# crowdbotp/socialways

Measured on AMD Instinct MI355X. Metric: GAN train steps/sec (256 scenes x 8 agents x 8+12 T per GPU step; fp32; social block on), higher is better.
Workload: dtype f32; 1 GPU; m1: 256 scenes x 8 agents x (8 obs + 12 pred) per GPU step = reference --batch-size 2048; use_social=True, n_unrolling_steps=1, info loss on; full=False, global_batch_scenes=256, parallelism=dp1, steps_per_graph_launch=32, settle_steps=992, rehearsal_regions=2, step_alg_bytes=5527040, inputs=z drawn on the host every step

## Files before the change

### socialways_amd/csrc/sw_disc.hip

```cpp
#include "../../include/socialways_hip.h"
#include "sw_lstm_dev.h"
#include "sw_wgrad.h"
#include "sw_wgrad_dev.h"
#include <cstdlib>
#ifdef SW_PHASE_STAMPS
__device__ long long sw_disc_stamps[16];
#define SW_STAMP(k) do { __builtin_amdgcn_sched_barrier(0); long long _t = clock64(); if (blockIdx.x == 0 && threadIdx.x == 0) sw_disc_stamps[k] += _t - _tprev; _tprev = _t; __builtin_amdgcn_sched_barrier(0); } while (0)
#define SW_STAMP_INIT long long _tprev = clock64()
extern "C" int sw_debug_disc_stamps(long long* out, int reset) {
  if (reset) { long long z[16] = {0}; return (int)hipMemcpyToSymbol(HIP_SYMBOL(sw_disc_stamps), z, sizeof(z)); }
  return (int)hipMemcpyFromSymbol(out, HIP_SYMBOL(sw_disc_stamps), 16 * sizeof(long long));
}
#else
#define SW_STAMP(k)
#define SW_STAMP_INIT
#endif

#define SW_DSTAMP(k) SW_STAMP(k)
#define SW_DSTAMP_INIT SW_STAMP_INIT
#include "sw_disc_dev.h"

__global__ __launch_bounds__(SW_THREADS, 2) void disc_fwd_kernel(
    const float* __restrict__ obsv, int To, int x_mode, const float* __restrict__ pred_a,
    const float* __restrict__ pred_b, int nb, const float* __restrict__ d_w, int B, int Tp, float* __restrict__ label_a, float* __restrict__ label_b,
    float* __restrict__ code_a, float* __restrict__ code_b, float* __restrict__ dsave, int save_lstm, int split,
    float* __restrict__ w_snap, int fuse, DiscLoss gl, float* __restrict__ dpred_out, const float* __restrict__ dimg) {
  extern __shared__ __attribute__((aligned(16))) float smem[];
  disc_fwd_tile(smem, blockIdx.x, gridDim.x, obsv, To, x_mode, pred_a, pred_b, nb, d_w, B, Tp, label_a, label_b, code_a, code_b, dsave,
                save_lstm, split, w_snap, fuse, gl, dpred_out, dimg);
}

#define SW_SPLIT_MAX_WGS 256

__global__ __launch_bounds__(SW_THREADS, 2) void disc_bwd_kernel(
    const float* __restrict__ d_w, const float* __restrict__ dsave, const float* __restrict__ dlabel_a,
    const float* __restrict__ dlabel_b, const float* __restrict__ dcode_a, const float* __restrict__ dcode_b, int nb,
    int B, int To, int Tp, int want_w, float* __restrict__ ddelta, float* __restrict__ dpred_a,
    float* __restrict__ dpred_b, DiscLoss gl, const float* __restrict__ dimg) {
  extern __shared__ __attribute__((aligned(16))) float smem[];
  const HeadLdsB L = head_lds_b(Tp, 0);
  float* dgbuf = smem + L.pe0T;
  const swp::Disc O = swp::disc(Tp);
  const DSave ds = dsave_layout(B, To, Tp, nb);
  const DDelta dd = ddelta_layout(B, To, Tp, nb);
  const int lane = sw_lane(), wave = sw_wave(), ln = lane & 15, lg = lane >> 4;
  const int u0 = wave * 16;
  const int a0 = blockIdx.x * SW_TILE;
  const int b = min(a0 + ln, B - 1);
  const bool live = (a0 + ln) < B;
  const int K4 = 4 * Tp;

  SW_STAMP_INIT;
  const int m0h = 16 * (wave & 1);
  f32x4 pc1[2], pq1[2], po1;
#pragma unroll
  for (int k = 0; k < 2; ++k) {
    const size_t kb = (size_t)min(k, nb - 1) * B + b;
    pc1[k] = ld4(dsave + (wave < 2 ? ds.c1 : ds.l1) + kb * 32 + m0h + 4 * lg);
    pq1[k] = ld4(dsave + ds.q1 + kb * 32 + m0h + 4 * lg);
  }
  po1 = ld4(dsave + ds.o1 + (size_t)b * 32 + m0h + 4 * lg);
  float hl[2][2], hc[2][2], hz[2], htg[2], rl[2], rc[2], rz[2];
  {
    const float* zsrc = gl.on ? gl.z : dsave;
    const float* tsrc = gl.on ? gl.targets : dsave;
    htg[0] = tsrc[gl.on ? gl.t0 : 0];
    htg[1] = tsrc[gl.on ? gl.t1 : 0];
    const float* dl1 = nb > 1 ? dlabel_b : dlabel_a;
    const float* dc1p = nb > 1 ? dcode_b : dcode_a;
#pragma unroll
    for (int e = 0; e < 2; ++e) {
      const int i = min((int)threadIdx.x + SW_THREADS * e, 16 * LD16 - 1);
      const int a = i / LD16, c1 = min(i - a * LD16, 1);
      const int bb = min(a0 + a, B - 1);
      hl[e][0] = dlabel_a[bb];
      hl[e][1] = dl1[bb];
      hc[e][0] = dcode_a[(size_t)bb * 2 + c1];
      hc[e][1] = dc1p[(size_t)bb * 2 + c1];
      hz[e] = zsrc[(size_t)bb * SW_Z + c1];
    }
    const int bb = min(a0 + ln, B - 1);
    rl[0] = dlabel_a[bb];
    rl[1] = dl1[bb];
    rc[0] = dcode_a[(size_t)bb * 2];
    rc[1] = dcode_a[(size_t)bb * 2 + 1];
    rz[0] = zsrc[(size_t)bb * SW_Z];
    rz[1] = zsrc[(size_t)bb * SW_Z + 1];
  }
  for (int i = threadIdx.x; i < 16 * LD32; i += blockDim.x) smem[L.docode + i] = 0.f;
  disc_stage_headT(smem, L, true, d_w, O, K4, dimg, true, [&] {
    stage_zero(smem + L.of0T, L.dlab - L.of0T);
    sw_barrier();
  });

  for (int k = 0; k < nb; ++k) {
    float* dpred = k == 0 ? dpred_a : dpred_b;
    sw_barrier();
    if (k == 0) SW_STAMP(8);
#pragma unroll
    for (int e = 0; e < 2; ++e) {
      const int i = threadIdx.x + SW_THREADS * e;
      if (i < 16 * LD16) {
        const int a = i / LD16, cc = i - a * LD16;
        const int bb = min(a0 + a, B - 1);
        const float xl = k == 0 ? hl[e][0] : hl[e][1], xc = k == 0 ? hc[e][0] : hc[e][1];
        float vl, vc;
        if (gl.on) {
          const float tgt = k == 0 ? htg[0] : htg[1];
          vl = cc == 0 ? 2.0f * (xl - tgt) * gl.g_label : 0.f;
          vc = (k == 0 && cc < 2) ? 2.0f * (xc - hz[e]) * gl.g_code : 0.f;
        } else {
          vl = cc == 0 ? xl : 0.f;
          vc = cc < 2 ? xc : 0.f;
        }
        smem[L.dlab + i] = vl;
        smem[L.dcod + i] = vc;
        if (want_w && a0 + a < B && cc < 4) {
          ddelta[dd.dlab + ((size_t)k * B + bb) * 4 + cc] = vl;
          ddelta[dd.dcod + ((size_t)k * B + bb) * 4 + cc] = vc;
        }
      }
    }
    if (gl.on && gl.loss_part && wave == 3 && k < 2) {
      const bool lv = lane < 16 && a0 + lane < B;
      const float e = (k == 0 ? rl[0] : rl[1]) - (k == 0 ? htg[0] : htg[1]);
      float sl = lv ? e * e : 0.f, sc = 0.f;
      if (k == 0 && lv) {
        const float c0 = rc[0] - rz[0], c1 = rc[1] - rz[1];
        sc = c0 * c0 + c1 * c1;
      }
#pragma unroll
      for (int o = 8; o > 0; o >>= 1) {
        sl += __shfl_xor(sl, o);
        sc += __shfl_xor(sc, o);
      }
      if (lane == 0) {
        gl.loss_part[(size_t)blockIdx.x * 3 + (k == 0 ? 0 : 2)] = sl;
        if (k == 0) gl.loss_part[(size_t)blockIdx.x * 3 + 1] = sc;
      }
    }
    sw_barrier();
    {
      int m0 = 16 * (wave & 1);
      bool cls = wave < 2;
      f32x4 acc = {0.f, 0.f, 0.f, 0.f};
      acc = tile_mm_rt(smem + (cls ? L.cl1T : L.la1T) + (m0 + ln) * LD16 + 4 * lg,
                       smem + (cls ? L.dlab : L.dcod) + ln * LD16 + 4 * lg, 1, acc);
      const f32x4 a = k == 0 ? pc1[0] : pc1[1];
#pragma unroll
      for (int r = 0; r < 4; ++r) acc[r] = sw_lrelu_grad(a[r], acc[r]);
      st4(smem + (cls ? L.dc1 : L.dl1) + ln * LD32 + m0 + 4 * lg, acc);
      if (want_w && live) st4(ddelta + (cls ? dd.dc1 : dd.dl1) + ((size_t)k * B + b) * 32 + m0 + 4 * lg, acc);
    }
    sw_barrier();
    {
      f32x4 acc = {0.f, 0.f, 0.f, 0.f};
      acc = tile_mm_rt(smem + L.cl0T + (u0 + ln) * LD32 + 4 * lg, smem + L.dc1 + ln * LD32 + 4 * lg, 2, acc);
      acc = tile_mm_rt(smem + L.la0T + (u0 + ln) * LD32 + 4 * lg, smem + L.dl1 + ln * LD32 + 4 * lg, 2, acc);
      st4(smem + L.dboth + ln * LD64 + u0 + 4 * lg, acc);
      if (wave < 2) {
        float* p = smem + L.docode + ln * LD32 + u0 + 4 * lg;
        st4(p, ld4(p) + acc);
      } else if (want_w && live) {
        st4(ddelta + dd.dpcode + ((size_t)k * B + b) * 32 + (u0 - 32) + 4 * lg, acc);
      }
    }
    sw_barrier();
    if (wave < 2) {
      int m0 = 16 * wave;
      f32x4 acc = {0.f, 0.f, 0.f, 0.f};
      acc = tile_mm_rt(smem + L.pe1T + (m0 + ln) * LD32 + 4 * lg, smem + L.dboth + ln * LD64 + 32 + 4 * lg, 2, acc);
      const f32x4 a = k == 0 ? pq1[0] : pq1[1];
#pragma unroll
      for (int r = 0; r < 4; ++r) acc[r] = sw_lrelu_grad(a[r], acc[r]);
      st4(smem + L.dq1 + ln * LD32 + m0 + 4 * lg, acc);
      if (want_w && live) st4(ddelta + dd.dq1 + ((size_t)k * B + b) * 32 + m0 + 4 * lg, acc);
    }
    sw_barrier();
    if (dpred) {
      for (int mt = wave; mt * 16 < K4; mt += 4) {
        int m0 = 16 * mt;
        f32x4 acc = {0.f, 0.f, 0.f, 0.f};
        acc = tile_mm_rt(smem + L.pe0T + (m0 + ln) * LD32 + 4 * lg, smem + L.dq1 + ln * LD32 + 4 * lg, 2, acc);
        if (live && m0 + 4 * lg < K4) st4(dpred + (size_t)b * K4 + m0 + 4 * lg, acc);
      }
    }
  }
  if (!want_w) return;
  sw_barrier();
  SW_STAMP(9);
  if (live && wave < 2) st4(ddelta + dd.docode + (size_t)b * 32 + u0 + 4 * lg, ld4(smem + L.docode + ln * LD32 + u0 + 4 * lg));
  f32x4 dh = disc_obs_bwd_tail(smem + L.of1T, smem + L.of0T, smem + L.docode, smem + L.do1, po1, ddelta + dd.do1 + (size_t)b * 32, live);
  f32x4 dc = {0.f, 0.f, 0.f, 0.f};
  LstmWT WT;
  lstm_load_whhT(WT, dimg, swdimg::OP_WHHT, d_w + O.whh, wave, lane);
  const LstmBptt S{dsave + ds.act + (size_t)b * 384 + u0 + 4 * lg, nullptr, dgbuf, ddelta + dd.dgates + (size_t)a0 * 256,
                   ddelta + dd.trash, a0, B};
  lstm_bptt_rows<false>(WT, S, To, dh, dc, SwNop{}, [&](int k) { SW_STAMP(k); });
}

namespace {
struct UpdLds {
  int hbuf, hw, bias, hwT, x, q1, both, c1, l1, o1, total;
  int dlab, dcod, dc1, dl1, dboth, docode, do1, dend;
  int ldp;
  HeadLds F;
  HeadLdsB T;
};
__host__ __device__ inline UpdLds upd_lds(int Tp) {
  UpdLds U;
  U.F = head_lds(Tp, 0);
  U.T = head_lds_b(Tp, 0);
  U.ldp = U.F.ldp;
  int o = 0;
  U.hbuf = o; o += 2 * 16 * SW_HLD;
  U.hw = o; o += U.F.bias - U.F.of0;
  U.bias = o; o += 8 * 32;
  U.hwT = o; o += U.T.dlab - U.T.of0T;
  U.x = o; o += 2 * 16 * U.ldp;
  U.q1 = o; o += 2 * 16 * LD32;
  U.both = o; o += 2 * 16 * LD64;
  U.c1 = o; o += 2 * 16 * LD32;
  U.l1 = o; o += 2 * 16 * LD32;
  U.o1 = o; o += 16 * LD32;
  U.total = o;
  int d = U.hw;
  U.dlab = d; d += 2 * 16 * LD16;
  U.dcod = d; d += 2 * 16 * LD16;
  U.dc1 = d; d += 2 * 16 * LD32;
  U.dl1 = d; d += 2 * 16 * LD32;
  U.dboth = d; d += 2 * 16 * LD64;
  U.docode = d; d += 16 * LD32;
  U.do1 = d; d += 16 * LD32;
  U.dend = d;
  return U;
}
}

__global__ __launch_bounds__(SW_THREADS) void disc_update_kernel(
    const float* __restrict__ obsv, int To, const float* __restrict__ pred_a, const float* __restrict__ pred_b,
    const float* __restrict__ d_w, int B, int Tp, float* __restrict__ label_a, float* __restrict__ label_b,
    float* __restrict__ code_a, float* __restrict__ code_b, float* __restrict__ dsave, int obs_pre, float* __restrict__ w_snap,
    DiscLoss gl, float* __restrict__ ddelta, const float* __restrict__ dimg) {
  extern __shared__ __attribute__((aligned(16))) float smem[];
  const UpdLds U = upd_lds(Tp);
  const HeadLds& F = U.F;
  const HeadLdsB& T = U.T;
  const swp::Disc O = swp::disc(Tp);
  const DSave ds = dsave_layout(B, To, Tp, 2);
  const DDelta dd = ddelta_layout(B, To, Tp, 2);
  float* hbuf = smem + U.hbuf;
  const int lane = sw_lane(), wave = sw_wave(), ln = lane & 15, lg = lane >> 4;
  const int u0 = wave * 16, br = wave >> 1, wp = wave & 1;
  const int a0 = blockIdx.x * SW_TILE;
  const int b = min(a0 + ln, B - 1);
  const bool live = (a0 + ln) < B;
  const int K4 = 4 * Tp, ldp = U.ldp;
  float* hw = smem + U.hw - F.of0;
  float* hwT = smem + U.hwT - T.of0T;

  float xpre[2][4];
  disc_xpre_load(xpre, pred_a, pred_b, a0, B, K4, ldp);
  const float tg0 = gl.targets[gl.t0], tg1 = gl.targets[gl.t1];
  const float z0 = gl.z[(size_t)b * SW_Z], z1 = gl.z[(size_t)b * SW_Z + 1];
  LstmW W;
  if (!obs_pre) disc_obs_operands(W, d_w, O, dimg);
  if (w_snap)
    for (int i = blockIdx.x * SW_THREADS + threadIdx.x; i < O.n; i += gridDim.x * SW_THREADS) w_snap[i] = d_w[i];
  disc_stage_heads(hw, F, d_w, O, K4, true);
  disc_stage_headT(hwT, T, true, nullptr, O, K4, dimg, false);
#pragma unroll
  for (int kk = 0; kk < 2; ++kk)
    disc_xpre_put(xpre, kk == 1, smem + U.x + kk * 16 * ldp, dsave + ds.px + (size_t)kk * B * K4, a0, B, K4, ldp);
  f32x4 c = {0.f, 0.f, 0.f, 0.f}, h = {0.f, 0.f, 0.f, 0.f};
  disc_seed_h(hbuf, obs_pre, dsave + ds.act, To, B, b);
  sw_barrier();
  const bool reg8 = !obs_pre && To == 8;
  f32x4 sg[8][4], sc[8];
  if (reg8) {
    float xa, xq;
    obs_x4_load(obsv, b, 0, 8, lg, xa, xq);
    asm volatile("" : "+v"(xa), "+v"(xq));
    float* hrow_g = dsave + ds.act + (size_t)b * 384 + 320 + u0 + 4 * lg;
    float* xrow = dsave + ds.x4s + (size_t)b * 4 + lg;
#pragma unroll
    for (int t = 0; t < 8; ++t) {
      const float xb = xa - (lg >= 2 ? xq : 0.f);
      obs_x4_load(obsv, b, t + 1 < 8 ? t + 1 : 7, 8, lg, xa, xq);
      lstm_cell(W, xb, &hbuf[(t & 1) * 16 * SW_HLD + ln * SW_HLD + 4 * lg], sg[t], c, h);
      sc[t] = c;
      st4(&hbuf[((t + 1) & 1) * 16 * SW_HLD + ln * SW_HLD + u0 + 4 * lg], h);
      st4g(hrow_g, h);
      *xrow = xb;
      hrow_g += (size_t)B * 384;
      xrow += (size_t)B * 4;
      sw_barrier();
      asm volatile("" : "+v"(xa), "+v"(xq));
    }
  } else if (!obs_pre) {
    lstm_obs_loop<0, true>(W, hbuf, obsv, To, B, b, c, h, dsave + ds.act, dsave + ds.x4s);
  }
  const float* hlast = &hbuf[(To & 1) * 16 * SW_HLD];

  const f32x4 o1reg = disc_obs_fc(hw, F, hlast, smem + U.o1, dsave + ds.o1 + (size_t)b * 32, live, smem + U.both, 2);
  float* xb_ = smem + U.x + br * 16 * ldp;
  float* q1_ = smem + U.q1 + br * 16 * LD32;
  float* both_ = smem + U.both + br * 16 * LD64;
  float* c1_ = smem + U.c1 + br * 16 * LD32;
  float* l1_ = smem + U.l1 + br * 16 * LD32;
  const size_t kb = (size_t)br * B + b;
  f32x4 q1reg, c1reg, l1reg;
  {
    const int m0 = 16 * wp;
    f32x4 acc = ld4(smem + U.bias + 2 * 32 + m0 + 4 * lg);
    acc = tile_mm_rt(hw + F.pe0 + (m0 + ln) * ldp + 4 * lg, xb_ + ln * ldp + 4 * lg, (ldp - 4) / 16, acc);
#pragma unroll
    for (int r = 0; r < 4; ++r) acc[r] = sw_lrelu(acc[r]);
    q1reg = acc;
    st4(q1_ + ln * LD32 + m0 + 4 * lg, acc);
    if (live) st4(dsave + ds.q1 + kb * 32 + m0 + 4 * lg, acc);
  }
  sw_barrier();
  {
    stage_zero(smem + U.dlab, U.dc1 - U.dlab);
    const int m0 = 16 * wp;
    f32x4 acc = ld4(smem + U.bias + 3 * 32 + m0 + 4 * lg);
    acc = tile_mm_rt(hw + F.pe1 + (m0 + ln) * LD32 + 4 * lg, q1_ + ln * LD32 + 4 * lg, 2, acc);
    st4(both_ + ln * LD64 + 32 + m0 + 4 * lg, acc);
  }
  sw_barrier();
  {
    if (live) {
      st4(dsave + ds.both + kb * 64 + 32 * wp + 4 * lg, ld4(both_ + ln * LD64 + 32 * wp + 4 * lg));
      st4(dsave + ds.both + kb * 64 + 32 * wp + 16 + 4 * lg, ld4(both_ + ln * LD64 + 32 * wp + 16 + 4 * lg));
    }
    const int m0 = 16 * wp;
    f32x4 ac = ld4(smem + U.bias + 4 * 32 + m0 + 4 * lg), al = ld4(smem + U.bias + 5 * 32 + m0 + 4 * lg);
    ac = tile_mm_rt(hw + F.cl0 + (m0 + ln) * LD64 + 4 * lg, both_ + ln * LD64 + 4 * lg, 4, ac);
    al = tile_mm_rt(hw + F.la0 + (m0 + ln) * LD64 + 4 * lg, both_ + ln * LD64 + 4 * lg, 4, al);
#pragma unroll
    for (int r = 0; r < 4; ++r) {
      ac[r] = sw_lrelu(ac[r]);
      al[r] = sw_lrelu(al[r]);
    }
    c1reg = ac;
    l1reg = al;
    st4(c1_ + ln * LD32 + m0 + 4 * lg, ac);
    st4(l1_ + ln * LD32 + m0 + 4 * lg, al);
    if (live) {
      st4(dsave + ds.c1 + kb * 32 + m0 + 4 * lg, ac);
      st4(dsave + ds.l1 + kb * 32 + m0 + 4 * lg, al);
    }
  }
  sw_barrier();
  {
    const bool cls = wp == 0;
    f32x4 acc = ld4(smem + U.bias + (cls ? 6 : 7) * 32 + 4 * lg);
    acc = tile_mm_rt(hw + (cls ? F.cl1 : F.la1) + ln * LD32 + 4 * lg, (cls ? c1_ : l1_) + ln * LD32 + 4 * lg, 2, acc);
    float* label = br == 0 ? label_a : label_b;
    float* code = br == 0 ? code_a : code_b;
    float sl = 0.f;
    if (lg == 0) {
      if (cls) {
        if (live) label[b] = acc[0];
        const float e = acc[0] - (br == 0 ? tg0 : tg1);
        const float g = 2.0f * e * gl.g_label;
        smem[U.dlab + br * 16 * LD16 + ln * LD16] = g;
        if (live) st4(ddelta + dd.dlab + kb * 4, f32x4{g, 0.f, 0.f, 0.f});
        sl = live ? e * e : 0.f;
      } else {
        if (live) { code[(size_t)b * 2] = acc[0]; code[(size_t)b * 2 + 1] = acc[1]; }
        const float e0 = acc[0] - z0, e1 = acc[1] - z1;
        const float g0 = br == 0 ? 2.0f * e0 * gl.g_code : 0.f, g1 = br == 0 ? 2.0f * e1 * gl.g_code : 0.f;
        smem[U.dcod + br * 16 * LD16 + ln * LD16] = g0;
        smem[U.dcod + br * 16 * LD16 + ln * LD16 + 1] = g1;
        if (live) st4(ddelta + dd.dcod + kb * 4, f32x4{g0, g1, 0.f, 0.f});
        sl = live ? e0 * e0 + e1 * e1 : 0.f;
      }
    }
#pragma unroll
    for (int o = 8; o > 0; o >>= 1) sl += __shfl_xor(sl, o);
    if (gl.loss_part && lane == 0) {
      if (cls) gl.loss_part[(size_t)blockIdx.x * 3 + (br == 0 ? 0 : 2)] = sl;
      else if (br == 0) gl.loss_part[(size_t)blockIdx.x * 3 + 1] = sl;
    }
  }
  sw_barrier();
  float* dlab_ = smem + U.dlab + br * 16 * LD16;
  float* dcod_ = smem + U.dcod + br * 16 * LD16;
  float* dc1_ = smem + U.dc1 + br * 16 * LD32;
  float* dl1_ = smem + U.dl1 + br * 16 * LD32;
  float* dboth_ = smem + U.dboth + br * 16 * LD64;
  {
    const int m0 = 16 * wp;
    f32x4 ac = {0.f, 0.f, 0.f, 0.f}, al = ac;
    ac = tile_mm_rt(hwT + T.cl1T + (m0 + ln) * LD16 + 4 * lg, dlab_ + ln * LD16 + 4 * lg, 1, ac);
    al = tile_mm_rt(hwT + T.la1T + (m0 + ln) * LD16 + 4 * lg, dcod_ + ln * LD16 + 4 * lg, 1, al);
#pragma unroll
    for (int r = 0; r < 4; ++r) {
      ac[r] = sw_lrelu_grad(c1reg[r], ac[r]);
      al[r] = sw_lrelu_grad(l1reg[r], al[r]);
    }
    st4(dc1_ + ln * LD32 + m0 + 4 * lg, ac);
    st4(dl1_ + ln * LD32 + m0 + 4 * lg, al);
    if (live) {
      st4(ddelta + dd.dc1 + kb * 32 + m0 + 4 * lg, ac);
      st4(ddelta + dd.dl1 + kb * 32 + m0 + 4 * lg, al);
    }
  }
  sw_barrier();
  {
#pragma unroll
    for (int q = 0; q < 2; ++q) {
      const int m0 = 16 * (2 * wp + q);
      f32x4 acc = {0.f, 0.f, 0.f, 0.f};
      acc = tile_mm_rt(hwT + T.cl0T + (m0 + ln) * LD32 + 4 * lg, dc1_ + ln * LD32 + 4 * lg, 2, acc);
      acc = tile_mm_rt(hwT + T.la0T + (m0 + ln) * LD32 + 4 * lg, dl1_ + ln * LD32 + 4 * lg, 2, acc);
      st4(dboth_ + ln * LD64 + m0 + 4 * lg, acc);
      if (wp == 1 && live) st4(ddelta + dd.dpcode + kb * 32 + (m0 - 32) + 4 * lg, acc);
    }
  }
  sw_barrier();
  {
    const int m0 = 16 * wp;
    f32x4 acc = {0.f, 0.f, 0.f, 0.f};
    acc = tile_mm_rt(hwT + T.pe1T + (m0 + ln) * LD32 + 4 * lg, dboth_ + ln * LD64 + 32 + 4 * lg, 2, acc);
#pragma unroll
    for (int r = 0; r < 4; ++r) acc[r] = sw_lrelu_grad(q1reg[r], acc[r]);
    if (live) st4(ddelta + dd.dq1 + kb * 32 + m0 + 4 * lg, acc);
  }
  if (wave < 2) {
    const int m0 = 16 * wave;
    const f32x4 v = ld4(smem + U.dboth + ln * LD64 + m0 + 4 * lg) + ld4(smem + U.dboth + 16 * LD64 + ln * LD64 + m0 + 4 * lg);
    st4(smem + U.docode + ln * LD32 + m0 + 4 * lg, v);
    if (live) st4(ddelta + dd.docode + (size_t)b * 32 + m0 + 4 * lg, v);
  }
  sw_barrier();
  f32x4 dh = disc_obs_bwd_tail(hwT + T.of1T, hwT + T.of0T, smem + U.docode, smem + U.do1, o1reg, ddelta + dd.do1 + (size_t)b * 32, live);
  f32x4 dc = {0.f, 0.f, 0.f, 0.f};
  LstmWT WT;
  lstm_load_whhT(WT, dimg, swdimg::OP_WHHT, nullptr, wave, lane);
  const LstmBptt S{dsave + ds.act + (size_t)b * 384 + u0 + 4 * lg, nullptr, hwT + T.pe0T, ddelta + dd.dgates + (size_t)a0 * 256,
                   ddelta + dd.trash, a0, B};
  if (reg8) {
    sw_barrier();
#pragma unroll
    for (int j = 0; j < 16; ++j) asm volatile("" : "+v"(WT.whhT[j]));
#pragma unroll
    for (int t = 7; t >= 1; --t) lstm_bptt_step<false, false, true>(WT, S, t, sg[t], sc[t], sc[t - 1], dh, dc);
    f32x4 c_1 = {0.f, 0.f, 0.f, 0.f};
    lstm_bptt_step<false, false, false>(WT, S, 0, sg[0], sc[0], c_1, dh, dc);
    return;
  }
  lstm_bptt_rows<false>(WT, S, To, dh, dc, SwNop{}, [](int k) {
    if (k == 10) sw_barrier();
  });
}

static int g_disc_fwd_lds = 0;

size_t sw_dsave_floats(int B, int To, int Tp, int nb) { return dsave_layout(B, To, Tp, nb).total; }
size_t sw_ddelta_floats(int B, int To, int Tp, int nb) { return ddelta_layout(B, To, Tp, nb).total; }

extern "C" int sw_disc_fwd(const float* obsv, int To, int x_mode, const float* const* pred4, int nb,
                           const float* d_w, int B, int Tp, float* const* label, float* const* code, float* dsave,
                           int save_lstm, float* w_snapshot, void* stream) {
  if (!obsv || !pred4 || !d_w || !label || !code || nb < 1 || nb > SW_DISC_MAXB || B < 0 || To < 1 || Tp < 1 ||
      (x_mode != 0 && x_mode != 1) || (x_mode == 0 && To < 2) || save_lstm < 0 || save_lstm > 2 || (save_lstm == 2 && !dsave))
    return SW_EARG;
  for (int k = 0; k < nb; ++k)
    if (!pred4[k] || !label[k] || !code[k]) return SW_EARG;
  if (Tp > 64) return SW_ESHAPE;
  if (B == 0) return SW_OK;
  int lds = head_lds(Tp, 2 * 16 * SW_HLD + 1280).total * 4;
  if (lds > 163840) return SW_ESHAPE;
  if (int rc = sw_set_lds((const void*)disc_fwd_kernel, lds, g_disc_fwd_lds)) return rc;
  const int tiles = (B + SW_TILE - 1) / SW_TILE;
  const int split = (nb == 2 && 2 * tiles <= SW_SPLIT_MAX_WGS) ? 1 : 0;
  SW_LAUNCH(disc_fwd_kernel, dim3(split ? 2 * tiles : tiles), dim3(SW_THREADS), lds, (hipStream_t)stream,
                     obsv, To, x_mode, pred4[0], nb > 1 ? pred4[1] : nullptr, nb, d_w, B, Tp, label[0],
                     nb > 1 ? label[1] : nullptr, code[0], nb > 1 ? code[1] : nullptr, dsave, save_lstm, split, w_snapshot, 0, DiscLoss{}, nullptr,
                     sw_disc_images_for(d_w, Tp).img);
  SW_CHECK_LAUNCH("disc_fwd_kernel");
  return SW_OK;
}

extern "C" int sw_disc_dpred(const float* obsv, int To, int x_mode, const float* pred4, const float* d_w, int B, int Tp,
                             const float* targets, int t_idx, const float* z, float g_label, float g_code,
                             float* dpred4, float* label, float* code, float* loss_part, void* stream) {
  if (!obsv || !pred4 || !d_w || !targets || !z || !dpred4 || B < 0 || To < 1 || Tp < 1 || t_idx < 0 ||
      (x_mode != 0 && x_mode != 1) || (x_mode == 0 && To < 2))
    return SW_EARG;
  if (Tp > 64) return SW_ESHAPE;
  if (B == 0) return SW_OK;
  const int lds = disc_dpred_lds(Tp);
  if (lds > 163840) return SW_ESHAPE;
  if (int rc = sw_set_lds((const void*)disc_fwd_kernel, lds, g_disc_fwd_lds)) return rc;
  DiscLoss gl{targets, z, t_idx, t_idx, g_label, g_code, 1, loss_part};
  const int tiles = (B + SW_TILE - 1) / SW_TILE;
  SW_LAUNCH(disc_fwd_kernel, dim3(tiles), dim3(SW_THREADS), lds, (hipStream_t)stream, obsv, To, x_mode, pred4,
                     (const float*)nullptr, 1, d_w, B, Tp, label, (float*)nullptr, code, (float*)nullptr, (float*)nullptr, 0, 0,
                     (float*)nullptr, 1, gl, dpred4, sw_disc_images_for(d_w, Tp).img);
  SW_CHECK_LAUNCH("disc_fwd_kernel");
  return SW_OK;
}

namespace {
struct ScoreLds {
  HeadLds F;
  int x, q1, both, c1, l1, total;
};
__host__ __device__ inline ScoreLds score_lds(int Tp) {
  ScoreLds S;
  S.F = head_lds(Tp, 2 * 16 * SW_HLD);
  int o = S.F.o1 + 16 * LD32;
  if (2 * 16 * S.F.ldp <= 32 * LD64) S.x = S.F.of0;
  else { S.x = o; o += 2 * 16 * S.F.ldp; }
  S.q1 = S.F.of1;
  S.both = o; o += 2 * 16 * LD64;
  S.c1 = o; o += 2 * 16 * LD32;
  S.l1 = o; o += 2 * 16 * LD32;
  S.total = o;
  return S;
}
}

template <bool RAGGED>
__global__ __launch_bounds__(SW_THREADS) void disc_score_kernel(
    const float* __restrict__ obsv, int To, int x_mode, const float* __restrict__ pred4, const float* __restrict__ d_w, int B, int K,
    int Tp, float* __restrict__ score, float* __restrict__ code, int tiles, int kgroups, const float* __restrict__ dimg,
    const int* __restrict__ obs_len) {
  extern __shared__ __attribute__((aligned(16))) float smem[];
  float* hbuf = smem;
  const ScoreLds S = score_lds(Tp);
  const HeadLds& F = S.F;
  const swp::Disc O = swp::disc(Tp);
  const int lane = sw_lane(), wave = sw_wave(), ln = lane & 15, lg = lane >> 4;
  const int br = wave >> 1, wp = wave & 1;
  const int kg = blockIdx.x / tiles;
  const int a0 = (blockIdx.x - kg * tiles) * SW_TILE;
  const int k_lo = (int)(((long long)kg * K) / kgroups), k_hi = (int)(((long long)(kg + 1) * K) / kgroups);
  const int b = min(a0 + ln, B - 1);
  const bool live = (a0 + ln) < B;
  const int K4 = 4 * Tp, ldp = F.ldp;
  const size_t draw = (size_t)B * K4;

  const bool x_pre = 16 * ldp <= 4 * SW_THREADS;
  float xpre[2][4];
  disc_xpre_load(xpre, pred4 + (size_t)k_lo * draw, pred4 + (size_t)min(k_lo + 1, k_hi - 1) * draw, a0, B, K4, ldp);
  LstmW W;
  disc_obs_operands(W, d_w, O, dimg);
  disc_stage_heads(smem, F, d_w, O, K4, 32 * (ldp >> 2) <= 2 * SW_THREADS);
  f32x4 c = {0.f, 0.f, 0.f, 0.f}, h = {0.f, 0.f, 0.f, 0.f};
  disc_seed_h(hbuf, false, nullptr, To, B, b);
  sw_barrier();
  if constexpr (RAGGED) {
    if (x_mode == 0) lstm_obs_loop_ragged<0>(W, hbuf, obsv, To, b, obs_start(obs_len, b, To, 0), c, h);
    else lstm_obs_loop_ragged<1>(W, hbuf, obsv, To, b, obs_start(obs_len, b, To, 1), c, h);
  } else {
    if (x_mode == 0) lstm_obs_loop<0, false>(W, hbuf, obsv, To, B, b, c, h, nullptr, nullptr);
    else lstm_obs_loop<1, false>(W, hbuf, obsv, To, B, b, c, h, nullptr, nullptr);
  }
  disc_obs_fc(smem, F, &hbuf[(To & 1) * 16 * SW_HLD], smem + F.o1, nullptr, live, smem + S.both, 2);

  float* x_ = smem + S.x + br * 16 * ldp;
  float* q1_ = smem + S.q1 + br * 16 * LD32;
  float* both_ = smem + S.both + br * 16 * LD64;
  float* c1_ = smem + S.c1 + br * 16 * LD32;
  float* l1_ = smem + S.l1 + br * 16 * LD32;
  const int m0 = 16 * wp;
  for (int k = k_lo; k < k_hi; k += 2) {
    const int k1 = min(k + 1, k_hi - 1);
    sw_barrier();
    if (x_pre) {
#pragma unroll
      for (int s = 0; s < 2; ++s) disc_xpre_put(xpre, s == 1, smem + S.x + s * 16 * ldp, nullptr, a0, B, K4, ldp);
      if (k + 2 < k_hi)
        disc_xpre_load(xpre, pred4 + (size_t)(k + 2) * draw, pred4 + (size_t)min(k + 3, k_hi - 1) * draw, a0, B, K4, ldp);
    } else {
      for (int i = threadIdx.x; i < 2 * 16 * ldp; i += SW_THREADS) {
        const int s = i / (16 * ldp), r = i - s * 16 * ldp;
        const int a = r / ldp, cc = r - a * ldp;
        smem[S.x + i] = cc < K4 ? pred4[(size_t)(s ? k1 : k) * draw + (size_t)min(a0 + a, B - 1) * K4 + cc] : 0.f;
      }
    }
    sw_barrier();
    {
      f32x4 acc = ld4(smem + F.bias + 2 * 32 + m0 + 4 * lg);
      acc = tile_mm_rt(smem + F.pe0 + (m0 + ln) * ldp + 4 * lg, x_ + ln * ldp + 4 * lg, (ldp - 4) / 16, acc);
#pragma unroll
      for (int r = 0; r < 4; ++r) acc[r] = sw_lrelu(acc[r]);
      st4(q1_ + ln * LD32 + m0 + 4 * lg, acc);
    }
    sw_barrier();
    {
      f32x4 acc = ld4(smem + F.bias + 3 * 32 + m0 + 4 * lg);
      acc = tile_mm_rt(smem + F.pe1 + (m0 + ln) * LD32 + 4 * lg, q1_ + ln * LD32 + 4 * lg, 2, acc);
      st4(both_ + ln * LD64 + 32 + m0 + 4 * lg, acc);
    }
    sw_barrier();
    {
      f32x4 ac = ld4(smem + F.bias + 4 * 32 + m0 + 4 * lg), al = ld4(smem + F.bias + 5 * 32 + m0 + 4 * lg);
      ac = tile_mm_rt(smem + F.cl0 + (m0 + ln) * LD64 + 4 * lg, both_ + ln * LD64 + 4 * lg, 4, ac);
      al = tile_mm_rt(smem + F.la0 + (m0 + ln) * LD64 + 4 * lg, both_ + ln * LD64 + 4 * lg, 4, al);
#pragma unroll
      for (int r = 0; r < 4; ++r) {
        ac[r] = sw_lrelu(ac[r]);
        al[r] = sw_lrelu(al[r]);
      }
// ... 243 lines not shown
```

### socialways_amd/csrc/sw_disc_dev.h

```cpp
#pragma once
#include "../../include/socialways_hip.h"
#include "sw_lstm_dev.h"
#ifndef SW_DSTAMP
#define SW_DSTAMP(k)
#define SW_DSTAMP_INIT
#endif

namespace {
constexpr int LD64 = sw_ld(64);
constexpr int LD32 = sw_ld(32);
constexpr int LD16 = sw_ld(16);
#define SW_DISC_MAXB 2

struct DSave {
  size_t act, x4s, o1, both, q1, c1, l1, px, total;
};
__host__ __device__ inline DSave dsave_layout(int B, int To, int Tp, int nb) {
  DSave d;
  size_t b = (size_t)B;
  d.act = 0;
  d.x4s = d.act + (size_t)To * b * 384;
  d.o1 = d.x4s + (size_t)To * b * 4;
  d.both = d.o1 + b * 32;
  d.q1 = d.both + nb * b * 64;
  d.c1 = d.q1 + nb * b * 32;
  d.l1 = d.c1 + nb * b * 32;
  d.px = d.l1 + nb * b * 32;
  d.total = d.px + nb * b * 4 * Tp;
  return d;
}
struct DDelta {
  size_t dgates, do1, docode, dpcode, dq1, dc1, dl1, dlab, dcod, trash, total;
};
__host__ __device__ inline DDelta ddelta_layout(int B, int To, int Tp, int nb) {
  DDelta d;
  size_t b = (size_t)B;
  d.dgates = 0;
  d.do1 = d.dgates + (size_t)To * b * 256;
  d.docode = d.do1 + b * 32;
  d.dpcode = d.docode + b * 32;
  d.dq1 = d.dpcode + nb * b * 32;
  d.dc1 = d.dq1 + nb * b * 32;
  d.dl1 = d.dc1 + nb * b * 32;
  d.dlab = d.dl1 + nb * b * 32;
  d.dcod = d.dlab + nb * b * 4;
  d.trash = d.dcod + nb * b * 4;
  d.total = d.trash + 16 * 256;
  return d;
}

__device__ __forceinline__ f32x4 tile_mm_rt(const float* wrow, const float* xrow, int KJ, f32x4 acc) {
  f32x4 acc1 = {0.f, 0.f, 0.f, 0.f};
  for (int j0 = 0; j0 < KJ; j0 += 4) {
    f32x4 a[4], b[4];
#pragma unroll
    for (int q = 0; q < 4; ++q) {
      if (j0 + q < KJ) {
        a[q] = ld4(wrow + 16 * (j0 + q));
        b[q] = ld4(xrow + 16 * (j0 + q));
      }
    }
#pragma unroll
    for (int q = 0; q < 4; ++q) {
      if (j0 + q < KJ) {
        acc = SW_MFMA(a[q][0], b[q][0], acc);
        acc1 = SW_MFMA(a[q][1], b[q][1], acc1);
        acc = SW_MFMA(a[q][2], b[q][2], acc);
        acc1 = SW_MFMA(a[q][3], b[q][3], acc1);
      }
    }
  }
  return acc + acc1;
}

struct HeadLds {
  int of0, of1, pe0, pe1, cl0, la0, cl1, la1, bias, hlast, o1, x, q1, both, c1, l1, total, ldp;
};
__host__ __device__ inline HeadLds head_lds(int Tp, int base) {
  HeadLds L;
  int KP = ((4 * Tp + 15) / 16) * 16;
  L.ldp = KP + 4;
  int o = base;
  L.of0 = o; o += 32 * LD64;
  L.of1 = o; o += 32 * LD32;
  L.pe0 = o; o += 32 * L.ldp;
  L.pe1 = o; o += 32 * LD32;
  L.cl0 = o; o += 32 * LD64;
  L.la0 = o; o += 32 * LD64;
  L.cl1 = o; o += 16 * LD32;
  L.la1 = o; o += 16 * LD32;
  L.bias = o; o += 8 * 32;
  L.hlast = o; o += 16 * LD64;
  L.o1 = o; o += 16 * LD32;
  if (16 * L.ldp <= 32 * LD64) L.x = L.of0;
  else { L.x = o; o += 16 * L.ldp; }
  L.q1 = o; o += 16 * LD32;
  L.both = o; o += 16 * LD64;
  L.c1 = o; o += 16 * LD32;
  L.l1 = o; o += 16 * LD32;
  L.total = o;
  return L;
}
}

namespace {
struct HeadLdsB {
  int of0T, of1T, pe0T, pe1T, cl0T, la0T, cl1T, la1T, dlab, dcod, dc1, dl1, dboth, docode, dq1, do1, total, kp;
};
__host__ __device__ inline HeadLdsB head_lds_b(int Tp, int base) {
  HeadLdsB L;
  L.kp = ((4 * Tp + 15) / 16) * 16;
  int o = base;
  L.of0T = o; o += 64 * LD32;
  L.of1T = o; o += 32 * LD32;
  L.pe0T = o; o += L.kp * LD32;
  L.pe1T = o; o += 32 * LD32;
  L.cl0T = o; o += 64 * LD32;
  L.la0T = o; o += 64 * LD32;
  L.cl1T = o; o += 32 * LD16;
  L.la1T = o; o += 32 * LD16;
  L.dlab = o; o += 16 * LD16;
  L.dcod = o; o += 16 * LD16;
  L.dc1 = o; o += 16 * LD32;
  L.dl1 = o; o += 16 * LD32;
  L.dboth = o; o += 16 * LD64;
  L.dq1 = o; o += 16 * LD32;
  L.docode = o; o += 16 * LD32;
  L.do1 = o; o += 16 * LD32;
  L.total = o;
  return L;
}
static_assert(7040 + 36 * 16 + 320 + 320 + 576 + 576 + 1088 + 576 >= 2 * 16 * SW_GLD, "dgates tiles fit the dead region");

__host__ __device__ inline int disc_dpred_lds(int Tp) {
  return head_lds_b(Tp, head_lds(Tp, 2 * 16 * SW_HLD + 1280).total).total * 4;
}
}

struct DiscLoss {
  const float* targets;
  const float* z;
  int t0, t1;
  float g_label, g_code;
  int on;
  float* loss_part;
};

__device__ __forceinline__ void disc_xpre_load(float (&xpre)[2][4], const float* p0, const float* p1, int a0, int B, int K4, int ldp) {
#pragma unroll
  for (int kk = 0; kk < 2; ++kk) {
    const float* pk = kk == 0 ? p0 : p1;
#pragma unroll
    for (int e = 0; e < 4; ++e) {
      const int i = min((int)threadIdx.x + SW_THREADS * e, 16 * ldp - 1);
      const int a = i / ldp, cc = i - a * ldp;
      xpre[kk][e] = pk[(size_t)min(a0 + a, B - 1) * K4 + min(cc, K4 - 1)];
    }
  }
}
__device__ __forceinline__ void disc_xpre_put(const float (&xpre)[2][4], bool s1, float* x, float* px, int a0, int B, int K4, int ldp) {
#pragma unroll
  for (int e = 0; e < 4; ++e) {
    const int i = threadIdx.x + SW_THREADS * e;
    if (i < 16 * ldp) {
      const int a = i / ldp, cc = i - a * ldp;
      const float v = cc < K4 ? (s1 ? xpre[1][e] : xpre[0][e]) : 0.f;
      x[i] = v;
      if (px && cc < K4 && a0 + a < B) px[(size_t)(a0 + a) * K4 + cc] = v;
    }
  }
}

__device__ __forceinline__ void disc_obs_operands(LstmW& W, const float* d_w, const swp::Disc& O, const float* dimg) {
  const int lane = sw_lane(), wave = sw_wave(), ln = lane & 15, lg = lane >> 4, u0 = wave * 16;
  if (!dimg) lstm_load_whh(W, d_w + O.whh, u0, ln, lg);
#pragma unroll
  for (int g = 0; g < 4; ++g) {
    if (dimg) {
#pragma unroll
      for (int j = 0; j < 4; ++j) W.whh[g][j] = ld4(dimg + swdimg::OP_WHH + ((((size_t)4 * g + wave) * 4 + j) * 64 + lane) * 4);
    }
    W.wx[g] = d_w[O.wih + (g * 64 + u0 + ln) * 4 + lg];
    W.bias[g] = ld4(d_w + O.bih + g * 64 + u0 + 4 * lg) + ld4(d_w + O.bhh + g * 64 + u0 + 4 * lg);
  }
}

__device__ __forceinline__ void disc_stage_heads(float* hw, const HeadLds& L, const float* d_w, const swp::Disc& O, int K4,
                                                 bool pe0_small) {
  f32x4 s_of0[3], s_of1[2], s_pe0[2], s_pe1[2], s_cl0[3], s_la0[3], s_cl1[1], s_la1[1];
  stage_w_load<3>(s_of0, LD64, 32, d_w + O.of0w, 64, 32, 64);
  stage_w_load<2>(s_of1, LD32, 32, d_w + O.of1w, 32, 32, 32);
  if (pe0_small) stage_w_load<2>(s_pe0, L.ldp, 32, d_w + O.pe0w, K4, 32, K4);
  stage_w_load<2>(s_pe1, LD32, 32, d_w + O.pe1w, 32, 32, 32);
  stage_w_load<3>(s_cl0, LD64, 32, d_w + O.cl0w, 64, 32, 64);
  stage_w_load<3>(s_la0, LD64, 32, d_w + O.la0w, 64, 32, 64);
  stage_w_load<1>(s_cl1, LD32, 16, d_w + O.cl1w, 32, 1, 32);
  stage_w_load<1>(s_la1, LD32, 16, d_w + O.la1w, 32, 2, 32);
  stage_w_store<3>(s_of0, hw + L.of0, LD64, 32);
  stage_w_store<2>(s_of1, hw + L.of1, LD32, 32);
  if (pe0_small) stage_w_store<2>(s_pe0, hw + L.pe0, L.ldp, 32);
  else stage_w(hw + L.pe0, L.ldp, 32, d_w + O.pe0w, K4, 32, K4);
  stage_w_store<2>(s_pe1, hw + L.pe1, LD32, 32);
  stage_w_store<3>(s_cl0, hw + L.cl0, LD64, 32);
  stage_w_store<3>(s_la0, hw + L.la0, LD64, 32);
  stage_w_store<1>(s_cl1, hw + L.cl1, LD32, 16);
  stage_w_store<1>(s_la1, hw + L.la1, LD32, 16);
  const int i = threadIdx.x;
  const int q = i >> 5, k = i & 31;
  const int boff = q == 0 ? O.of0b : q == 1 ? O.of1b : q == 2 ? O.pe0b : q == 3 ? O.pe1b : q == 4 ? O.cl0b
                   : q == 5 ? O.la0b : q == 6 ? O.cl1b : O.la1b;
  const int lim = q < 6 ? 32 : (q == 6 ? 1 : 2);
  const float v = d_w[boff + min(k, lim - 1)];
  hw[L.bias + i] = k < lim ? v : 0.f;
}

template <class Between = SwNop>
__device__ __forceinline__ void disc_stage_headT(float* base, const HeadLdsB& L, bool obs, const float* d_w, const swp::Disc& O,
                                                 int K4, const float* dimg, bool tail, Between between = {}) {
  const int from = obs ? L.of0T : L.pe0T;
  if (dimg || !d_w) {
    constexpr int HB = 12;
    const int n4 = (L.dlab - from) >> 2;
    const float* src = dimg + swdimg::HEADT + (from - L.of0T);
// ... 261 lines not shown
```

Before: 2747 steps/s.

## Restructure disc update head to chain layers in registers and cut barriers

Rewrites the discriminator update kernel's head forward/backward so that consecutive small matmuls feed their outputs directly from registers (new tile_mm_rb helper) instead of round-tripping through LDS with a barrier between each layer. Work is reassigned across waves (wave 0 does the obs FC chain, waves 1-2 do the pred chain; each wave computes a whole 32-wide layer), removing several sw_barrier calls and LDS buffers (dlab, dcod, c1, l1, docode, do1) and the barrier before BPTT. The obs backward tail is computed redundantly per wave rather than shared through LDS. It also adds optional phase timestamps for profiling. Risks: less parallelism per layer and redundant work in some waves, plus more register pressure.

```diff
diff --git a/socialways_amd/csrc/sw_disc.hip b/socialways_amd/csrc/sw_disc.hip
--- a/socialways_amd/csrc/sw_disc.hip
+++ b/socialways_amd/csrc/sw_disc.hip
@@ -4,16 +4,18 @@
 #include "sw_wgrad_dev.h"
 #include <cstdlib>
 #ifdef SW_PHASE_STAMPS
-__device__ long long sw_disc_stamps[16];
+__device__ long long sw_disc_stamps[64];
 #define SW_STAMP(k) do { __builtin_amdgcn_sched_barrier(0); long long _t = clock64(); if (blockIdx.x == 0 && threadIdx.x == 0) sw_disc_stamps[k] += _t - _tprev; _tprev = _t; __builtin_amdgcn_sched_barrier(0); } while (0)
 #define SW_STAMP_INIT long long _tprev = clock64()
 extern "C" int sw_debug_disc_stamps(long long* out, int reset) {
-  if (reset) { long long z[16] = {0}; return (int)hipMemcpyToSymbol(HIP_SYMBOL(sw_disc_stamps), z, sizeof(z)); }
-  return (int)hipMemcpyFromSymbol(out, HIP_SYMBOL(sw_disc_stamps), 16 * sizeof(long long));
-}
+  if (reset) { long long z[64] = {0}; return (int)hipMemcpyToSymbol(HIP_SYMBOL(sw_disc_stamps), z, sizeof(z)); }
+  return (int)hipMemcpyFromSymbol(out, HIP_SYMBOL(sw_disc_stamps), 64 * sizeof(long long));
+}
+#define SW_USTAMP(k) SW_STAMP((obs_pre ? 16 : 32) + (k))
 #else
 #define SW_STAMP(k)
 #define SW_STAMP_INIT
+#define SW_USTAMP(k)
 #endif
 
 #define SW_DSTAMP(k) SW_STAMP(k)
@@ -201,8 +203,8 @@
 
 namespace {
 struct UpdLds {
-  int hbuf, hw, bias, hwT, x, q1, both, c1, l1, o1, total;
-  int dlab, dcod, dc1, dl1, dboth, docode, do1, dend;
+  int hbuf, hw, bias, hwT, x, q1, both, o1, total;
+  int dc1, dl1, dboth, dend;
   int ldp;
   HeadLds F;
   HeadLdsB T;
@@ -220,18 +222,12 @@
   U.x = o; o += 2 * 16 * U.ldp;
   U.q1 = o; o += 2 * 16 * LD32;
   U.both = o; o += 2 * 16 * LD64;
-  U.c1 = o; o += 2 * 16 * LD32;
-  U.l1 = o; o += 2 * 16 * LD32;
   U.o1 = o; o += 16 * LD32;
   U.total = o;
   int d = U.hw;
-  U.dlab = d; d += 2 * 16 * LD16;
-  U.dcod = d; d += 2 * 16 * LD16;
   U.dc1 = d; d += 2 * 16 * LD32;
   U.dl1 = d; d += 2 * 16 * LD32;
-  U.dboth = d; d += 2 * 16 * LD64;
-  U.docode = d; d += 16 * LD32;
-  U.do1 = d; d += 16 * LD32;
+  U.dboth = d; d += 2 * 16 * LD32;
   U.dend = d;
   return U;
 }
@@ -258,6 +254,7 @@
   const int K4 = 4 * Tp, ldp = U.ldp;
   float* hw = smem + U.hw - F.of0;
   float* hwT = smem + U.hwT - T.of0T;
+  SW_STAMP_INIT;
 
   float xpre[2][4];
   disc_xpre_load(xpre, pred_a, pred_b, a0, B, K4, ldp);
@@ -275,6 +272,7 @@
   f32x4 c = {0.f, 0.f, 0.f, 0.f}, h = {0.f, 0.f, 0.f, 0.f};
   disc_seed_h(hbuf, obs_pre, dsave + ds.act, To, B, b);
   sw_barrier();
+  SW_USTAMP(0);
   const bool reg8 = !obs_pre && To == 8;
   f32x4 sg[8][4], sc[8];
   if (reg8) {
@@ -301,79 +299,97 @@
     lstm_obs_loop<0, true>(W, hbuf, obsv, To, B, b, c, h, dsave + ds.act, dsave + ds.x4s);
   }
   const float* hlast = &hbuf[(To & 1) * 16 * SW_HLD];
-
-  const f32x4 o1reg = disc_obs_fc(hw, F, hlast, smem + U.o1, dsave + ds.o1 + (size_t)b * 32, live, smem + U.both, 2);
-  float* xb_ = smem + U.x + br * 16 * ldp;
-  float* q1_ = smem + U.q1 + br * 16 * LD32;
+  SW_USTAMP(1);
+
   float* both_ = smem + U.both + br * 16 * LD64;
-  float* c1_ = smem + U.c1 + br * 16 * LD32;
-  float* l1_ = smem + U.l1 + br * 16 * LD32;
+  float* dc1_ = smem + U.dc1 + br * 16 * LD32;
+  float* dl1_ = smem + U.dl1 + br * 16 * LD32;
   const size_t kb = (size_t)br * B + b;
-  f32x4 q1reg, c1reg, l1reg;
+  const f32x4 zero4 = {0.f, 0.f, 0.f, 0.f};
+  if (wave == 0) {
+    f32x4 o1r[2];
+#pragma unroll
+    for (int t = 0; t < 2; ++t) {
+      const int m0 = 16 * t;
+      f32x4 acc = ld4(smem + U.bias + 0 * 32 + m0 + 4 * lg);
+      acc = tile_mm_rt(hw + F.of0 + (m0 + ln) * LD64 + 4 * lg, hlast + ln * SW_HLD + 4 * lg, 4, acc);
+#pragma unroll
+      for (int r = 0; r < 4; ++r) acc[r] = sw_lrelu(acc[r]);
+      o1r[t] = acc;
+      st4(smem + U.o1 + ln * LD32 + m0 + 4 * lg, acc);
+      if (live) st4(dsave + ds.o1 + (size_t)b * 32 + m0 + 4 * lg, acc);
+    }
+#pragma unroll
+    for (int t = 0; t < 2; ++t) {
+      const int m0 = 16 * t;
+      f32x4 acc = ld4(smem + U.bias + 1 * 32 + m0 + 4 * lg);
+      acc = tile_mm_rb<2>(hw + F.of1 + (m0 + ln) * LD32 + 4 * lg, o1r, acc);
+      st4(smem + U.both + ln * LD64 + m0 + 4 * lg, acc);
+      st4(smem + U.both + 16 * LD64 + ln * LD64 + m0 + 4 * lg, acc);
+    }
+  } else if (wave < 3) {
+    const int k = wave - 1;
+    const float* xk = smem + U.x + k * 16 * ldp;
+    const size_t kbk = (size_t)k * B + b;
+    f32x4 q1r[2];
+#pragma unroll
+    for (int t = 0; t < 2; ++t) {
+      const int m0 = 16 * t;
+      f32x4 acc = ld4(smem + U.bias + 2 * 32 + m0 + 4 * lg);
+      acc = tile_mm_rt(hw + F.pe0 + (m0 + ln) * ldp + 4 * lg, xk + ln * ldp + 4 * lg, (ldp - 4) / 16, acc);
+#pragma unroll
+      for (int r = 0; r < 4; ++r) acc[r] = sw_lrelu(acc[r]);
+      q1r[t] = acc;
+      st4(smem + U.q1 + k * 16 * LD32 + ln * LD32 + m0 + 4 * lg, acc);
+      if (live) st4(dsave + ds.q1 + kbk * 32 + m0 + 4 * lg, acc);
+    }
+#pragma unroll
+    for (int t = 0; t < 2; ++t) {
+      const int m0 = 16 * t;
+      f32x4 acc = ld4(smem + U.bias + 3 * 32 + m0 + 4 * lg);
+      acc = tile_mm_rb<2>(hw + F.pe1 + (m0 + ln) * LD32 + 4 * lg, q1r, acc);
+      st4(smem + U.both + k * 16 * LD64 + ln * LD64 + 32 + m0 + 4 * lg, acc);
+    }
+  }
+  sw_barrier();
+  SW_USTAMP(2);
   {
-    const int m0 = 16 * wp;
-    f32x4 acc = ld4(smem + U.bias + 2 * 32 + m0 + 4 * lg);
-    acc = tile_mm_rt(hw + F.pe0 + (m0 + ln) * ldp + 4 * lg, xb_ + ln * ldp + 4 * lg, (ldp - 4) / 16, acc);
-#pragma unroll
-    for (int r = 0; r < 4; ++r) acc[r] = sw_lrelu(acc[r]);
-    q1reg = acc;
-    st4(q1_ + ln * LD32 + m0 + 4 * lg, acc);
-    if (live) st4(dsave + ds.q1 + kb * 32 + m0 + 4 * lg, acc);
-  }
-  sw_barrier();
-  {
-    stage_zero(smem + U.dlab, U.dc1 - U.dlab);
-    const int m0 = 16 * wp;
-    f32x4 acc = ld4(smem + U.bias + 3 * 32 + m0 + 4 * lg);
-    acc = tile_mm_rt(hw + F.pe1 + (m0 + ln) * LD32 + 4 * lg, q1_ + ln * LD32 + 4 * lg, 2, acc);
-    st4(both_ + ln * LD64 + 32 + m0 + 4 * lg, acc);
-  }
-  sw_barrier();
-  {
+    const bool cls = wp == 0;
     if (live) {
       st4(dsave + ds.both + kb * 64 + 32 * wp + 4 * lg, ld4(both_ + ln * LD64 + 32 * wp + 4 * lg));
       st4(dsave + ds.both + kb * 64 + 32 * wp + 16 + 4 * lg, ld4(both_ + ln * LD64 + 32 * wp + 16 + 4 * lg));
     }
-    const int m0 = 16 * wp;
-    f32x4 ac = ld4(smem + U.bias + 4 * 32 + m0 + 4 * lg), al = ld4(smem + U.bias + 5 * 32 + m0 + 4 * lg);
-    ac = tile_mm_rt(hw + F.cl0 + (m0 + ln) * LD64 + 4 * lg, both_ + ln * LD64 + 4 * lg, 4, ac);
-    al = tile_mm_rt(hw + F.la0 + (m0 + ln) * LD64 + 4 * lg, both_ + ln * LD64 + 4 * lg, 4, al);
-#pragma unroll
-    for (int r = 0; r < 4; ++r) {
-      ac[r] = sw_lrelu(ac[r]);
-      al[r] = sw_lrelu(al[r]);
-    }
-    c1reg = ac;
-    l1reg = al;
-    st4(c1_ + ln * LD32 + m0 + 4 * lg, ac);
-    st4(l1_ + ln * LD32 + m0 + 4 * lg, al);
-    if (live) {
-      st4(dsave + ds.c1 + kb * 32 + m0 + 4 * lg, ac);
-      st4(dsave + ds.l1 + kb * 32 + m0 + 4 * lg, al);
-    }
-  }
-  sw_barrier();
-  {
-    const bool cls = wp == 0;
+    f32x4 a1r[2];
+#pragma unroll
+    for (int t = 0; t < 2; ++t) {
+      const int m0 = 16 * t;
+      f32x4 acc = ld4(smem + U.bias + (cls ? 4 : 5) * 32 + m0 + 4 * lg);
+      acc = tile_mm_rt(hw + (cls ? F.cl0 : F.la0) + (m0 + ln) * LD64 + 4 * lg, both_ + ln * LD64 + 4 * lg, 4, acc);
+#pragma unroll
+      for (int r = 0; r < 4; ++r) acc[r] = sw_lrelu(acc[r]);
+      a1r[t] = acc;
+      if (live) st4(dsave + (cls ? ds.c1 : ds.l1) + kb * 32 + m0 + 4 * lg, acc);
+    }
     f32x4 acc = ld4(smem + U.bias + (cls ? 6 : 7) * 32 + 4 * lg);
-    acc = tile_mm_rt(hw + (cls ? F.cl1 : F.la1) + ln * LD32 + 4 * lg, (cls ? c1_ : l1_) + ln * LD32 + 4 * lg, 2, acc);
+    acc = tile_mm_rb<2>(hw + (cls ? F.cl1 : F.la1) + ln * LD32 + 4 * lg, a1r, acc);
     float* label = br == 0 ? label_a : label_b;
     float* code = br == 0 ? code_a : code_b;
     float sl = 0.f;
+    f32x4 dout[1] = {zero4};
     if (lg == 0) {
       if (cls) {
         if (live) label[b] = acc[0];
         const float e = acc[0] - (br == 0 ? tg0 : tg1);
         const float g = 2.0f * e * gl.g_label;
-        smem[U.dlab + br * 16 * LD16 + ln * LD16] = g;
+        dout[0][0] = g;
         if (live) st4(ddelta + dd.dlab + kb * 4, f32x4{g, 0.f, 0.f, 0.f});
         sl = live ? e * e : 0.f;
       } else {
         if (live) { code[(size_t)b * 2] = acc[0]; code[(size_t)b * 2 + 1] = acc[1]; }
         const float e0 = acc[0] - z0, e1 = acc[1] - z1;
         const float g0 = br == 0 ? 2.0f * e0 * gl.g_code : 0.f, g1 = br == 0 ? 2.0f * e1 * gl.g_code : 0.f;
-        smem[U.dcod + br * 16 * LD16 + ln * LD16] = g0;
-        smem[U.dcod + br * 16 * LD16 + ln * LD16 + 1] = g1;
+        dout[0][0] = g0;
+        dout[0][1] = g1;
         if (live) st4(ddelta + dd.dcod + kb * 4, f32x4{g0, g1, 0.f, 0.f});
         sl = live ? e0 * e0 + e1 * e1 : 0.f;
       }
@@ -384,77 +400,82 @@
       if (cls) gl.loss_part[(size_t)blockIdx.x * 3 + (br == 0 ? 0 : 2)] = sl;
       else if (br == 0) gl.loss_part[(size_t)blockIdx.x * 3 + 1] = sl;
     }
+#pragma unroll
+    for (int t = 0; t < 2; ++t) {
+      const int m0 = 16 * t;
+      f32x4 d = tile_mm_rb<1>(hwT + (cls ? T.cl1T : T.la1T) + (m0 + ln) * LD16 + 4 * lg, dout, zero4);
+#pragma unroll
+      for (int r = 0; r < 4; ++r) d[r] = sw_lrelu_grad(a1r[t][r], d[r]);
+      st4((cls ? dc1_ : dl1_) + ln * LD32 + m0 + 4 * lg, d);
+      if (live) st4(ddelta + (cls ? dd.dc1 : dd.dl1) + kb * 32 + m0 + 4 * lg, d);
+    }
   }
   sw_barrier();
-  float* dlab_ = smem + U.dlab + br * 16 * LD16;
-  float* dcod_ = smem + U.dcod + br * 16 * LD16;
-  float* dc1_ = smem + U.dc1 + br * 16 * LD32;
-  float* dl1_ = smem + U.dl1 + br * 16 * LD32;
-  float* dboth_ = smem + U.dboth + br * 16 * LD64;
+  SW_USTAMP(3);
   {
-    const int m0 = 16 * wp;
-    f32x4 ac = {0.f, 0.f, 0.f, 0.f}, al = ac;
-    ac = tile_mm_rt(hwT + T.cl1T + (m0 + ln) * LD16 + 4 * lg, dlab_ + ln * LD16 + 4 * lg, 1, ac);
-    al = tile_mm_rt(hwT + T.la1T + (m0 + ln) * LD16 + 4 * lg, dcod_ + ln * LD16 + 4 * lg, 1, al);
-#pragma unroll
-    for (int r = 0; r < 4; ++r) {
-      ac[r] = sw_lrelu_grad(c1reg[r], ac[r]);
-      al[r] = sw_lrelu_grad(l1reg[r], al[r]);
-    }
-    st4(dc1_ + ln * LD32 + m0 + 4 * lg, ac);
-    st4(dl1_ + ln * LD32 + m0 + 4 * lg, al);
-    if (live) {
-      st4(ddelta + dd.dc1 + kb * 32 + m0 + 4 * lg, ac);
-      st4(ddelta + dd.dl1 + kb * 32 + m0 + 4 * lg, al);
-    }
-  }
-  sw_barrier();
-  {
+    f32x4 dbr[2];
 #pragma unroll
     for (int q = 0; q < 2; ++q) {
       const int m0 = 16 * (2 * wp + q);
-      f32x4 acc = {0.f, 0.f, 0.f, 0.f};
+      f32x4 acc = zero4;
       acc = tile_mm_rt(hwT + T.cl0T + (m0 + ln) * LD32 + 4 * lg, dc1_ + ln * LD32 + 4 * lg, 2, acc);
       acc = tile_mm_rt(hwT + T.la0T + (m0 + ln) * LD32 + 4 * lg, dl1_ + ln * LD32 + 4 * lg, 2, acc);
-      st4(dboth_ + ln * LD64 + m0 + 4 * lg, acc);
-      if (wp == 1 && live) st4(ddelta + dd.dpcode + kb * 32 + (m0 - 32) + 4 * lg, acc);
+      dbr[q] = acc;
+      if (wp == 0) st4(smem + U.dboth + br * 16 * LD32 + ln * LD32 + m0 + 4 * lg, acc);
+      else if (live) st4(ddelta + dd.dpcode + kb * 32 + (m0 - 32) + 4 * lg, acc);
+    }
+    if (wp == 1) {
+#pragma unroll
+      for (int t = 0; t < 2; ++t) {
+        const int m0 = 16 * t;
+        f32x4 d = tile_mm_rb<2>(hwT + T.pe1T + (m0 + ln) * LD32 + 4 * lg, dbr, zero4);
+        const f32x4 q1v = ld4(smem + U.q1 + br * 16 * LD32 + ln * LD32 + m0 + 4 * lg);
+#pragma unroll
+        for (int r = 0; r < 4; ++r) d[r] = sw_lrelu_grad(q1v[r], d[r]);
+        if (live) st4(ddelta + dd.dq1 + kb * 32 + m0 + 4 * lg, d);
+      }
     }
   }
   sw_barrier();
+  SW_USTAMP(4);
+  f32x4 dh;
   {
-    const int m0 = 16 * wp;
-    f32x4 acc = {0.f, 0.f, 0.f, 0.f};
-    acc = tile_mm_rt(hwT + T.pe1T + (m0 + ln) * LD32 + 4 * lg, dboth_ + ln * LD64 + 32 + 4 * lg, 2, acc);
-#pragma unroll
-    for (int r = 0; r < 4; ++r) acc[r] = sw_lrelu_grad(q1reg[r], acc[r]);
-    if (live) st4(ddelta + dd.dq1 + kb * 32 + m0 + 4 * lg, acc);
-  }
-  if (wave < 2) {
-    const int m0 = 16 * wave;
-    const f32x4 v = ld4(smem + U.dboth + ln * LD64 + m0 + 4 * lg) + ld4(smem + U.dboth + 16 * LD64 + ln * LD64 + m0 + 4 * lg);
-    st4(smem + U.docode + ln * LD32 + m0 + 4 * lg, v);
-    if (live) st4(ddelta + dd.docode + (size_t)b * 32 + m0 + 4 * lg, v);
-  }
-  sw_barrier();
-  f32x4 dh = disc_obs_bwd_tail(hwT + T.of1T, hwT + T.of0T, smem + U.docode, smem + U.do1, o1reg, ddelta + dd.do1 + (size_t)b * 32, live);
+    f32x4 docr[2], do1r[2];
+#pragma unroll
+    for (int t = 0; t < 2; ++t)
+      docr[t] = ld4(smem + U.dboth + ln * LD32 + 16 * t + 4 * lg) + ld4(smem + U.dboth + 16 * LD32 + ln * LD32 + 16 * t + 4 * lg);
+#pragma unroll
+    for (int t = 0; t < 2; ++t) {
+      f32x4 d = tile_mm_rb<2>(hwT + T.of1T + (16 * t + ln) * LD32 + 4 * lg, docr, zero4);
+      const f32x4 o1v = ld4(smem + U.o1 + ln * LD32 + 16 * t + 4 * lg);
+#pragma unroll
+      for (int r = 0; r < 4; ++r) d[r] = sw_lrelu_grad(o1v[r], d[r]);
+      do1r[t] = d;
+    }
+    if (wave < 2 && live) {
+      st4(ddelta + dd.docode + (size_t)b * 32 + u0 + 4 * lg, wave == 0 ? docr[0] : docr[1]);
+      st4(ddelta + dd.do1 + (size_t)b * 32 + u0 + 4 * lg, wave == 0 ? do1r[0] : do1r[1]);
+    }
+    dh = tile_mm_rb<2>(hwT + T.of0T + (u0 + ln) * LD32 + 4 * lg, do1r, zero4);
+  }
+  SW_USTAMP(5);
   f32x4 dc = {0.f, 0.f, 0.f, 0.f};
   LstmWT WT;
   lstm_load_whhT(WT, dimg, swdimg::OP_WHHT, nullptr, wave, lane);
   const LstmBptt S{dsave + ds.act + (size_t)b * 384 + u0 + 4 * lg, nullptr, hwT + T.pe0T, ddelta + dd.dgates + (size_t)a0 * 256,
                    ddelta + dd.trash, a0, B};
   if (reg8) {
-    sw_barrier();
 #pragma unroll
     for (int j = 0; j < 16; ++j) asm volatile("" : "+v"(WT.whhT[j]));
 #pragma unroll
     for (int t = 7; t >= 1; --t) lstm_bptt_step<false, false, true>(WT, S, t, sg[t], sc[t], sc[t - 1], dh, dc);
     f32x4 c_1 = {0.f, 0.f, 0.f, 0.f};
     lstm_bptt_step<false, false, false>(WT, S, 0, sg[0], sc[0], c_1, dh, dc);
+    SW_USTAMP(6);
     return;
   }
-  lstm_bptt_rows<false>(WT, S, To, dh, dc, SwNop{}, [](int k) {
-    if (k == 10) sw_barrier();
-  });
+  lstm_bptt_rows<false>(WT, S, To, dh, dc);
+  SW_USTAMP(6);
 }
 
 static int g_disc_fwd_lds = 0;
diff --git a/socialways_amd/csrc/sw_disc_dev.h b/socialways_amd/csrc/sw_disc_dev.h
--- a/socialways_amd/csrc/sw_disc_dev.h
+++ b/socialways_amd/csrc/sw_disc_dev.h
@@ -69,6 +69,23 @@
         acc1 = SW_MFMA(a[q][3], b[q][3], acc1);
       }
     }
+  }
+  return acc + acc1;
+}
+
+template <int KJ>
+__device__ __forceinline__ f32x4 tile_mm_rb(const float* wrow, const f32x4 (&b)[KJ], f32x4 acc) {
+  static_assert(KJ >= 1 && KJ <= 4, "one group of k-steps");
+  f32x4 acc1 = {0.f, 0.f, 0.f, 0.f};
+  f32x4 a[KJ];
+#pragma unroll
+  for (int q = 0; q < KJ; ++q) a[q] = ld4(wrow + 16 * q);
+#pragma unroll
+  for (int q = 0; q < KJ; ++q) {
+    acc = SW_MFMA(a[q][0], b[q][0], acc);
+    acc1 = SW_MFMA(a[q][1], b[q][1], acc1);
+    acc = SW_MFMA(a[q][2], b[q][2], acc);
+    acc1 = SW_MFMA(a[q][3], b[q][3], acc1);
   }
   return acc + acc1;
 }
```

Result: no change. 2764 steps/s (median of 6 runs) (+0.6%).
